# DearCaat/MHIM-MIL

Measured on AMD Instinct MI355X. Metric: patch-instances/sec through MHIM fwd+bwd, N=10k D=1024, higher is better.
Workload: dtype f32; 1 GPU; c2: MHIM(ABMIL) train step, one bag N=10000 D=1024 per GPU per step (teacher fwd + select + student fwd + bwd + Adam + EMA); rotating_bags_per_gpu=8, matrix_core_form=bf16x3, parallelism=dp1, launch=hipGraph replay, one graph per resident bag

## Files before the change

### mhim_mil_amd/csrc/select.hip

```cpp
#include "select_dev.hpp"

namespace mhimx {

#ifdef MHIMX_SEL_PROF
__device__ unsigned long long sel_prof[32];
#define SEL_STAMP(i) do { __syncthreads(); if (threadIdx.x == 0) sel_prof[i] = wall_clock64(); } while (0)
#else
#define SEL_STAMP(i)
#endif


template <bool VOTE>
__global__ __launch_bounds__(SEL_THREADS) void select_kernel(
    const float* __restrict__ score_all, int64_t N, int k, int n_sel, int largest, const int64_t* __restrict__ perm,
    const int64_t* __restrict__ other, int64_t n_other, int64_t* __restrict__ mask_ids,
    int64_t* __restrict__ len_keep_dev, int64_t* __restrict__ topk_out, uint8_t* __restrict__ flags,
    float* __restrict__ vote, int P ) {
  extern __shared__ __attribute__((aligned(16))) char smem_raw[];
  uint64_t* keys = reinterpret_cast<uint64_t*>(smem_raw);
  uint32_t* hist = reinterpret_cast<uint32_t*>(keys + P);
  uint32_t* wave_tot = hist + SEL_WAVES * 256;
  uint32_t* misc = wave_tot + SEL_WAVES;
  const int tid = threadIdx.x, lane = tid & 63, wave = tid >> 6;
  const float* score = score_all + (VOTE ? (int64_t)blockIdx.x * N : 0);
// ... 22 lines not shown
  uint32_t prefix = mx, remaining = (uint32_t)k;
  if (mn != mx) {
    const int hb = 31 - __clz(mn ^ mx);
    uint32_t fixed_mask = hb >= 31 ? 0u : ~((2u << hb) - 1u);
    prefix = mx & fixed_mask;
    int shift = hb - 7 < 0 ? 0 : hb - 7;
    while (true) {
      for (int i = tid; i < SEL_WAVES * 256; i += SEL_THREADS) hist[i] = 0;
      __syncthreads();
      for (int64_t i = tid; i < N; i += SEL_THREADS) {
        const uint32_t key = mono32(score[i], lg);
        if ((key & fixed_mask) == prefix) atomicAdd(&hist[wave * 256 + ((key >> shift) & 255u)], 1u);
      }
      __syncthreads();
      if (tid < 256) {
        uint32_t c = 0;
#pragma unroll
        for (int w = 0; w < SEL_WAVES; ++w) c += hist[w * 256 + tid];
        hist[tid] = c;
      }
      __syncthreads();
      if (tid == 0) {
        uint32_t above = 0;
        int d = 255;
        for (; d > 0; --d) {
          if (above + hist[d] >= remaining) break;
          above += hist[d];
        }
        misc[0] = (uint32_t)d;
        misc[1] = remaining - above;
      }
      __syncthreads();
      prefix |= misc[0] << shift;
      remaining = misc[1];
      fixed_mask |= 0xFFu << shift;
      __syncthreads();
      if (shift == 0) break;
      shift = shift - 8 < 0 ? 0 : shift - 8;
    }
  }
  const uint32_t T = prefix;

  if (tid == 0) misc[2] = 0;
  __syncthreads();
  uint32_t eq_base = 0;
  for (int64_t c0 = 0; c0 < N; c0 += SEL_THREADS) {
    const int64_t i = c0 + tid;
    uint32_t key = 0;
    bool gt = false, eq = false;
    if (i < N) {
      key = mono32(score[i], lg);
      gt = key > T;
      eq = key == T;
    }
    uint32_t tot;
    const uint32_t rank = block_prefix(eq, wave_tot, &tot);
    const bool take = gt || (eq && (eq_base + rank) < remaining);
    if (take) {
      const uint32_t pos = atomicAdd(&misc[2], 1u);
      keys[pos] = ((uint64_t)key << 32) | (uint64_t)(0xFFFFFFFFu - (uint32_t)i);
    }
    eq_base += tot;
  }
  __syncthreads();

  if (VOTE) {
    for (int j = tid; j < k; j += SEL_THREADS) {
      const uint32_t idx = 0xFFFFFFFFu - (uint32_t)(keys[j] & 0xFFFFFFFFull);
      atomicAdd(&vote[idx], 1.0f);
    }
    return;
  }

  for (int j = k + tid; j < P; j += SEL_THREADS) keys[j] = 0ull;
  __syncthreads();
  for (int size = 2; size <= P; size <<= 1) {
    for (int stride = size >> 1; stride > 0; stride >>= 1) {
      for (int t = tid; t < (P >> 1); t += SEL_THREADS) {
        const int lo = 2 * t - (t & (stride - 1));
        const int hi = lo + stride;
        const bool desc = ((lo & size) == 0);
        const uint64_t a = keys[lo], b = keys[hi];
        if ((a < b) == desc) { keys[lo] = b; keys[hi] = a; }
      }
      __syncthreads();
    }
  }
  if (topk_out)
    for (int j = tid; j < k; j += SEL_THREADS) topk_out[j] = (int64_t)(0xFFFFFFFFu - (uint32_t)(keys[j] & 0xFFFFFFFFull));

  for (int64_t i = tid; i < N; i += SEL_THREADS) flags[i] = 0;
  __syncthreads();
  const bool has_other = other != nullptr && n_other > 0;
  const int64_t len_keep_simple = N - n_sel;
  for (int j = tid; j < n_sel; j += SEL_THREADS) {
    const int64_t src = perm ? perm[j] : (int64_t)j;
    const int64_t idx = (int64_t)(0xFFFFFFFFu - (uint32_t)(keys[src] & 0xFFFFFFFFull));
    flags[idx] = 1;
    if (!has_other) mask_ids[len_keep_simple + j] = idx;
  }
  if (has_other)
    for (int64_t j = tid; j < n_other; j += SEL_THREADS) flags[other[j]] = 1;
  __threadfence_block();
  __syncthreads();

  uint32_t kept_base = 0;
  for (int64_t c0 = 0; c0 < N; c0 += SEL_THREADS) {
    const int64_t i = c0 + tid;
    const bool keep = (i < N) && flags[i] == 0;
    uint32_t tot;
    const uint32_t rank = block_prefix(keep, wave_tot, &tot);
    if (keep) mask_ids[kept_base + rank] = i;
    kept_base += tot;
  }
  if (has_other) {
    uint32_t m_base = 0;
    for (int64_t c0 = 0; c0 < N; c0 += SEL_THREADS) {
      const int64_t i = c0 + tid;
      const bool msk = (i < N) && flags[i] != 0;
      uint32_t tot;
      const uint32_t rank = block_prefix(msk, wave_tot, &tot);
      if (msk) mask_ids[kept_base + m_base + rank] = i;
      m_base += tot;
    }
  }
  if (tid == 0 && len_keep_dev) *len_keep_dev = (int64_t)kept_base;
}



template <int KPT, bool LEAN = false>
__global__ __launch_bounds__(SEL_THREADS) void select_small_kernel(
    const float* __restrict__ score, int N, int k, int n_sel, int largest, const int64_t* __restrict__ perm,
    const int64_t* __restrict__ other, int64_t n_other, int64_t* __restrict__ mask_ids, int64_t* __restrict__ len_keep_dev,
    int64_t* __restrict__ topk_out, int P, int use_rand, uint64_t rand_seed0, const uint64_t* __restrict__ tick, int merge_R,
    int64_t* __restrict__ rows_out,
    int64_t* __restrict__ rows_img ,
    int img_off, BagBatch bb ) {
  extern __shared__ __attribute__((aligned(16))) char smem_raw[];
  if (blockIdx.z) {
    MHIMX_BAG(score); MHIMX_BAG(perm); MHIMX_BAG(other); MHIMX_BAG(mask_ids); MHIMX_BAG(len_keep_dev); MHIMX_BAG(topk_out); MHIMX_BAG(rows_out);
    MHIMX_BAG(rows_img);
    rand_seed0 = bag_sel_seed(rand_seed0, bb);
  }
  const uint64_t rand_seed = eff_seed(rand_seed0, tick);
  uint64_t* keys = reinterpret_cast<uint64_t*>(smem_raw);
  uint64_t* sorted = keys + P;
  uint32_t* hist = reinterpret_cast<uint32_t*>(sorted + P);
  uint32_t* wave_tot = hist + SEL_COPIES * SEL_BINS;
  uint32_t* misc = wave_tot + SEL_WAVES;
  uint32_t* bitmap = misc + 8;
  uint32_t* rank = bitmap + 512;
  uint16_t* klist = reinterpret_cast<uint16_t*>(rank + P);
  uint16_t* stage = reinterpret_cast<uint16_t*>(smem_raw);
  const int tid = threadIdx.x;
  const bool lg = largest != 0;
  const int i0 = tid * KPT;

  SEL_STAMP(8);
  uint32_t key[KPT];
  bool valid[KPT];
#pragma unroll
  for (int j = 0; j < KPT; ++j) {
    valid[j] = (i0 + j) < N;
    key[j] = valid[j] ? mono32(score[i0 + j], lg) : 0u;
  }
  SEL_STAMP(0);
  for (int i = tid; i < 512; i += SEL_THREADS) bitmap[i] = 0;
  if (tid == 0) misc[2] = 0;

  uint32_t remaining, n_eq;
  const uint32_t T = radix_select_regs<KPT, false>(key, valid, (uint32_t)k, hist, wave_tot, misc, &remaining, &n_eq);

  SEL_STAMP(1);
  uint32_t eq_rank = 0;
  if (remaining != n_eq) {
    uint32_t neq = 0;
#pragma unroll
    for (int j = 0; j < KPT; ++j) neq += (valid[j] && key[j] == T) ? 1u : 0u;
    uint32_t tot;
    eq_rank = block_scan_excl(neq, wave_tot, &tot);
  }
  bool take[KPT];
  uint32_t ntake = 0;
#pragma unroll
  for (int j = 0; j < KPT; ++j) {
    bool t = valid[j] && key[j] > T;
    if (valid[j] && key[j] == T) { t = remaining == n_eq || eq_rank < remaining; ++eq_rank; }
    take[j] = t;
    ntake += t ? 1u : 0u;
  }
  {
    uint32_t tot;
    uint32_t pos = block_scan_excl(ntake, wave_tot, &tot);
#pragma unroll
    for (int j = 0; j < KPT; ++j)
      if (take[j]) keys[pos++] = ((uint64_t)key[j] << 32) | (uint64_t)(0xFFFFFFFFu - (uint32_t)(i0 + j));
  }
  __syncthreads();

  SEL_STAMP(2);
  const bool dev_rand = LEAN || (use_rand && !perm && n_sel < k);
  const uint64_t* cand = keys;
  if (LEAN || (dev_rand && !topk_out)) {
  } else if (k <= 2048) {
    for (int j = tid; j < k; j += SEL_THREADS) {
      const uint64_t mine = keys[j];
      int r = 0;
      for (int q = 0; q < k; ++q) r += keys[q] > mine ? 1 : 0;
      sorted[r] = mine;
    }
    __syncthreads();
  } else {
    for (int j = tid; j < P; j += SEL_THREADS) sorted[j] = j < k ? keys[j] : 0ull;
    __syncthreads();
    for (int size = 2; size <= P; size <<= 1)
      for (int stride = size >> 1; stride > 0; stride >>= 1) {
        for (int t = tid; t < (P >> 1); t += SEL_THREADS) {
          const int lo = 2 * t - (t & (stride - 1)), hi = lo + stride;
          const bool desc = ((lo & size) == 0);
          const uint64_t a = sorted[lo], b = sorted[hi];
          if ((a < b) == desc) { sorted[lo] = b; sorted[hi] = a; }
        }
        __syncthreads();
      }
  }
  if (!LEAN && topk_out)
    for (int j = tid; j < k; j += SEL_THREADS) topk_out[j] = (int64_t)(0xFFFFFFFFu - (uint32_t)(sorted[j] & 0xFFFFFFFFull));

  SEL_STAMP(3);
  const bool has_other = !LEAN && other != nullptr && n_other > 0;
  const int len_keep_simple = N - n_sel;
  if (dev_rand) {
    const uint32_t k0 = mix32((uint32_t)rand_seed ^ 0x9E3779B9u), k1 = mix32((uint32_t)(rand_seed >> 32) + 0x85EBCA6Bu + k0 * 0x632BE5ABu);
    const int bits = small_perm_bits((uint32_t)k);
    for (int i = tid; i < n_sel; i += SEL_THREADS) {
      const uint32_t j = feistel_small((uint32_t)i, (uint32_t)k, bits, k0, k1);
      const uint32_t idx = 0xFFFFFFFFu - (uint32_t)(cand[j] & 0xFFFFFFFFull);
      atomicOr(&bitmap[idx >> 5], 1u << (idx & 31));
      if (!LEAN && !has_other && mask_ids) mask_ids[len_keep_simple + i] = (int64_t)idx;
    }
  } else if (!LEAN) {
    for (int j = tid; j < n_sel; j += SEL_THREADS) {
      const int64_t src = perm ? perm[j] : (int64_t)j;
      const uint32_t idx = 0xFFFFFFFFu - (uint32_t)(sorted[src] & 0xFFFFFFFFull);
      atomicOr(&bitmap[idx >> 5], 1u << (idx & 31));
      if (!has_other && mask_ids) mask_ids[len_keep_simple + j] = (int64_t)idx;
    }
  }
  if (has_other)
    for (int64_t j = tid; j < n_other; j += SEL_THREADS) {
      const uint32_t idx = (uint32_t)other[j];
      atomicOr(&bitmap[idx >> 5], 1u << (idx & 31));
    }
  __syncthreads();

  SEL_STAMP(4);
  bool kv[KPT];
  uint32_t nkeep = 0;
#pragma unroll
  for (int j = 0; j < KPT; ++j) {
    const int i = i0 + j;
    kv[j] = valid[j] && !((bitmap[i >> 5] >> (i & 31)) & 1u);
    nkeep += kv[j] ? 1u : 0u;
  }
  uint32_t kept_total;
  uint32_t kpos = block_scan_excl(nkeep, wave_tot, &kept_total);
  const uint32_t kpos0 = kpos;
  if (!LEAN && mask_ids) {
#pragma unroll
    for (int j = 0; j < KPT; ++j)
      if (kv[j]) mask_ids[kpos++] = i0 + j;
    if (has_other) {
      uint32_t nm = 0;
#pragma unroll
      for (int j = 0; j < KPT; ++j) nm += (valid[j] && !kv[j]) ? 1u : 0u;
      uint32_t mt;
      uint32_t mpos = kept_total + block_scan_excl(nm, wave_tot, &mt);
#pragma unroll
      for (int j = 0; j < KPT; ++j)
        if (valid[j] && !kv[j]) mask_ids[mpos++] = i0 + j;
    }
  }
  if (!LEAN && tid == 0 && len_keep_dev) *len_keep_dev = (int64_t)kept_total;
  SEL_STAMP(5);
  if (!LEAN && !rows_out) return;

  const int Lrows = (int)kept_total;
  const int Lk = Lrows - merge_R;
  const bool partial = merge_R > 0 && merge_R < Lrows;
  if (partial) {
    uint32_t kp = kpos0;
#pragma unroll
    for (int j = 0; j < KPT; ++j)
      if (kv[j]) klist[kp++] = (uint16_t)(i0 + j);
    for (int i = tid; i < 512; i += SEL_THREADS) bitmap[i] = 0;
    __syncthreads();
    const uint32_t q1 = mix32((uint32_t)rand_seed * 0x9E3779B1u + 0xC2B2AE35u), q0 = mix32(((uint32_t)(rand_seed >> 17) ^ 0x85EBCA6Bu) + q1 * 0x632BE5ABu);
    const int bits2 = small_perm_bits((uint32_t)Lrows);
    for (int i = tid; i < merge_R; i += SEL_THREADS) {
      const uint32_t row = klist[feistel_small((uint32_t)i, (uint32_t)Lrows, bits2, q0, q1)];
      atomicOr(&bitmap[row >> 5], 1u << (row & 31));
    }
    __syncthreads();
  }
  SEL_STAMP(6);
  bool mrg[KPT];
  uint32_t nstay = 0, nmrg = 0;
#pragma unroll
  for (int j = 0; j < KPT; ++j) {
    const int i = i0 + j;
    const bool m = kv[j] && (merge_R >= Lrows || (partial && ((bitmap[i >> 5] >> (i & 31)) & 1u)));
    mrg[j] = m;
    nmrg += m ? 1u : 0u;
    nstay += (kv[j] && !m) ? 1u : 0u;
  }
  uint32_t t2;
  const uint32_t packed = block_scan_excl(nstay | (nmrg << 16), wave_tot, &t2);
  uint32_t spos = (use_rand == 2 ? (uint32_t)(Lrows - Lk) : 0u) + (packed & 0xFFFFu);
  uint32_t mpos2 = (use_rand == 2 ? 0u : (uint32_t)Lk) + (packed >> 16);
  SEL_STAMP(10);
#pragma unroll
  for (int j = 0; j < KPT; ++j) {
    if (!kv[j]) continue;
    if (mrg[j]) stage[mpos2++] = (uint16_t)(i0 + j);
    else stage[spos++] = (uint16_t)(i0 + j);
  }
  __syncthreads();
  for (int i = tid; i < Lrows; i += SEL_THREADS) rows_out[i] = (int64_t)stage[i];
  if (rows_img) {
    const int mrg_n = Lrows - Lk, stay0 = use_rand == 2 ? mrg_n : 0, mrg0 = use_rand == 2 ? 0 : Lk;
    const int end = (img_off + mrg_n + 31) / 32 * 32;
    for (int p = tid; p < end; p += SEL_THREADS)
      rows_img[p] = p < Lk ? (int64_t)stage[stay0 + p] : ((p >= img_off && p - img_off < mrg_n) ? (int64_t)stage[mrg0 + p - img_off] : (int64_t)0);
  }
  SEL_STAMP(7);
}


constexpr int SELM_MAXG = 256;
__global__ void sel_zero_kernel(uint4* __restrict__ p, int64_t n16) {
  for (int64_t i = (int64_t)blockIdx.x * blockDim.x + threadIdx.x; i < n16; i += (int64_t)gridDim.x * blockDim.x) p[i] = make_uint4(0u, 0u, 0u, 0u);
}
static int sel_zero(hipStream_t st, void* p, int64_t bytes) {
  const int64_t n16 = bytes / 16;
  int64_t blocks = cdiv(n16, 256);
  if (blocks > 1024) blocks = 1024;
  hipLaunchKernelGGL(sel_zero_kernel, dim3((unsigned)blocks), dim3(256), 0, st, (uint4*)p, n16);
  return 0;
}
struct SelMultiWs {
  uint32_t* hist;
  uint32_t* rank;
  uint32_t* selpos;
  uint32_t* blk_gt;
  uint32_t* blk_eq;
  uint32_t* blk_keep;
  uint32_t* blk_mask;
  uint32_t* state;
  uint64_t* cand;
  uint8_t* flags;
};


template <int PASS>
__global__ __launch_bounds__(SEL_THREADS) void selm_hist_kernel(const float* __restrict__ score, int64_t N, int largest, int k, SelMultiWs w) {
  __shared__ uint32_t lh[SELM_BINS];
  __shared__ __attribute__((aligned(16))) uint32_t wave_tot[SEL_WAVES];
  __shared__ uint32_t misc[8];
  const int tid = threadIdx.x;
  const bool lg = largest != 0;
  uint32_t prefix = 0, rem = 0;
  selm_prefix(w.hist, PASS, (uint32_t)k, wave_tot, misc, &prefix, &rem);
  const uint32_t fixed_mask = PASS == 0 ? 0u : (PASS == 1 ? 0xFFE00000u : 0xFFFFFC00u);
  const int shift = PASS == 0 ? 21 : (PASS == 1 ? 10 : 0);
  const uint32_t dmask = PASS == 2 ? 1023u : 2047u;
  for (int i = tid; i < SELM_BINS; i += SEL_THREADS) lh[i] = 0;
  __syncthreads();
  for (int64_t i = (int64_t)blockIdx.x * SEL_THREADS + tid; i < N; i += (int64_t)gridDim.x * SEL_THREADS) {
    const uint32_t key = mono32(score[i], lg);
    if ((key & fixed_mask) == prefix) atomicAdd(&lh[(key >> shift) & dmask], 1u);
  }
  __syncthreads();
  uint32_t* gh = w.hist + PASS * SELM_BINS;
  for (int i = tid; i < SELM_BINS; i += SEL_THREADS)
    if (lh[i]) atomicAdd(&gh[i], lh[i]);
}

__global__ __launch_bounds__(SEL_THREADS) void selm_count_kernel(const float* __restrict__ score, int64_t N, int largest, int k, int64_t chunk,
                                                                SelMultiWs w) {
  __shared__ __attribute__((aligned(16))) uint32_t wave_tot[SEL_WAVES];
  __shared__ uint32_t misc[8];
  const int tid = threadIdx.x;
  const bool lg = largest != 0;
  uint32_t T, remaining;
  selm_prefix(w.hist, 3, (uint32_t)k, wave_tot, misc, &T, &remaining);
  if (blockIdx.x == 0 && tid == 0) { w.state[0] = T; w.state[1] = remaining; }
  const int64_t b0 = (int64_t)blockIdx.x * chunk, b1 = b0 + chunk < N ? b0 + chunk : N;
  uint32_t gt = 0, eq = 0;
  for (int64_t i = b0 + tid; i < b1; i += SEL_THREADS) {
    const uint32_t key = mono32(score[i], lg);
    gt += key > T ? 1u : 0u;
    eq += key == T ? 1u : 0u;
  }
  uint32_t tg, te;
  block_scan_excl(gt, wave_tot, &tg);
  block_scan_excl(eq, wave_tot, &te);
  if (tid == 0) { w.blk_gt[blockIdx.x] = tg; w.blk_eq[blockIdx.x] = te; }
}

__global__ __launch_bounds__(SEL_THREADS) void selm_gather_kernel(const float* __restrict__ score, int64_t N, int largest, int64_t chunk,
                                                                 SelMultiWs w) {
  __shared__ __attribute__((aligned(16))) uint32_t wave_tot[SEL_WAVES];
  __shared__ uint32_t misc[8];
  const int tid = threadIdx.x, b = blockIdx.x;
  const bool lg = largest != 0;
  const uint32_t T = w.state[0], remaining = w.state[1];
  if (tid == 0) {
    uint32_t eqb = 0, pos = 0;
    for (int q = 0; q < b; ++q) {
      const uint32_t e = w.blk_eq[q];
      const uint32_t room = remaining > eqb ? remaining - eqb : 0u;
      pos += w.blk_gt[q] + (e < room ? e : room);
      eqb += e;
    }
    misc[0] = eqb;
    misc[1] = pos;
  }
  __syncthreads();
  uint32_t eq_base = misc[0], pos_base = misc[1];
  __syncthreads();
  const int64_t b0 = (int64_t)b * chunk, b1 = b0 + chunk < N ? b0 + chunk : N;
  for (int64_t c0 = b0; c0 < b1; c0 += SEL_THREADS) {
    const int64_t i = c0 + tid;
    uint32_t key = 0;
    bool gt = false, eq = false;
    if (i < b1) {
      key = mono32(score[i], lg);
      gt = key > T;
      eq = key == T;
    }
    uint32_t tot_eq, tot_take;
    const uint32_t erank = block_prefix(eq, wave_tot, &tot_eq);
    const bool take = gt || (eq && (eq_base + erank) < remaining);
    const uint32_t trank = block_prefix(take, wave_tot, &tot_take);
    if (take) w.cand[pos_base + trank] = ((uint64_t)key << 32) | (uint64_t)(0xFFFFFFFFu - (uint32_t)i);
    eq_base += tot_eq;
    pos_base += tot_take;
  }
}

constexpr int SELM_SEG = 256;
__global__ __launch_bounds__(SEL_THREADS) void selm_rank_kernel(int k, int n_sel, const int64_t* __restrict__ perm, SelMultiWs w) {
  __shared__ uint64_t seg[SELM_SEG];
  const int tid = threadIdx.x;
  const int s0 = blockIdx.y * SELM_SEG;
  for (int i = tid; i < SELM_SEG; i += SEL_THREADS) seg[i] = (s0 + i) < k ? w.cand[s0 + i] : 0ull;
  if (blockIdx.y == 0) {
    for (int j = blockIdx.x * SEL_THREADS + tid; j < n_sel; j += gridDim.x * SEL_THREADS) w.selpos[perm ? perm[j] : (int64_t)j] = (uint32_t)j + 1u;
  }
  __syncthreads();
  const int j = blockIdx.x * SEL_THREADS + tid;
  if (j >= k) return;
  const uint64_t mine = w.cand[j];
  uint32_t r = 0;
#pragma unroll 8
  for (int q = 0; q < SELM_SEG; ++q) r += seg[q] > mine ? 1u : 0u;
  if (r) atomicAdd(&w.rank[j], r);
// ... 233 lines not shown
```

### mhim_mil_amd/csrc/select_dev.hpp

```cpp
#pragma once
#include "common.hpp"

namespace mhimx {

constexpr int SEL_THREADS = 1024;
constexpr int SEL_WAVES = SEL_THREADS / 64;

MHIMX_DEV uint32_t mono32(float f, bool largest) {
  uint32_t b = __float_as_uint(f);
  b = (b & 0x80000000u) ? ~b : (b | 0x80000000u);
  return largest ? b : ~b;
}

MHIMX_DEV uint32_t block_prefix(bool pred, uint32_t* wave_tot , uint32_t* total) {
  const int lane = threadIdx.x & 63, wave = threadIdx.x >> 6;
  const unsigned long long bal = __ballot(pred);
  const uint32_t in_wave = __popcll(bal & ((1ull << lane) - 1ull));
  if (lane == 0) wave_tot[wave] = __popcll(bal);
  __syncthreads();
  uint32_t base = 0, tot = 0;
#pragma unroll
  for (int w = 0; w < SEL_WAVES; ++w) {
    const uint32_t c = wave_tot[w];
    if (w < wave) base += c;
// ... 12 lines not shown
  v += dpp_u32<0x111, 0xf>(0u, v);
  v += dpp_u32<0x112, 0xf>(0u, v);
  v += dpp_u32<0x114, 0xf>(0u, v);
  v += dpp_u32<0x118, 0xf>(0u, v);
  v += dpp_u32<0x142, 0xa>(0u, v);
  v += dpp_u32<0x143, 0xc>(0u, v);
  return v;
}
MHIMX_DEV uint32_t wave_min_u32(uint32_t v) {
  uint32_t t;
  t = dpp_u32<0xB1, 0xf>(v, v); v = t < v ? t : v;
  t = dpp_u32<0x4E, 0xf>(v, v); v = t < v ? t : v;
  t = dpp_u32<0x141, 0xf>(v, v); v = t < v ? t : v;
  t = dpp_u32<0x140, 0xf>(v, v); v = t < v ? t : v;
  t = dpp_u32<0x142, 0xa>(v, v); v = t < v ? t : v;
  t = dpp_u32<0x143, 0xc>(v, v); v = t < v ? t : v;
  return (uint32_t)__builtin_amdgcn_readlane((int)v, 63);
}
MHIMX_DEV uint32_t wave_max_u32(uint32_t v) { return ~wave_min_u32(~v); }

MHIMX_DEV void wave_tot_combine(const uint32_t* wave_tot, int wave, uint32_t* below, uint32_t* total) {
  uint32_t w[SEL_WAVES];
#pragma unroll
  for (int q = 0; q < SEL_WAVES / 4; ++q) {
    const uint4 v = reinterpret_cast<const uint4*>(wave_tot)[q];
    w[4 * q] = v.x; w[4 * q + 1] = v.y; w[4 * q + 2] = v.z; w[4 * q + 3] = v.w;
  }
  uint32_t b = 0, t = 0;
#pragma unroll
  for (int q = 0; q < SEL_WAVES; ++q) {
    b += q < wave ? w[q] : 0u;
    t += w[q];
  }
  *below = b;
  *total = t;
}

MHIMX_DEV uint32_t block_scan_excl(uint32_t v, uint32_t* wave_tot , uint32_t* total) {
  const int lane = threadIdx.x & 63, wave = threadIdx.x >> 6;
  const uint32_t inc = wave_scan_incl(v);
  if (lane == 63) wave_tot[wave] = inc;
  __syncthreads();
  uint32_t base;
  wave_tot_combine(wave_tot, wave, &base, total);
  __syncthreads();
  return base + inc - v;
}

constexpr int SEL_DIGIT = 11, SEL_BINS = 1 << SEL_DIGIT, SEL_COPIES = 4, SEL_LIST = 1024;

template <int KPT, bool FULL32>
MHIMX_DEV uint32_t radix_select_regs(const uint32_t (&key)[KPT], const bool (&valid)[KPT], uint32_t k, uint32_t* hist,
                                     uint32_t* wave_tot, uint32_t* misc, uint32_t* remaining_out, uint32_t* n_eq_out) {
  const int tid = threadIdx.x, wave = tid >> 6, lane = tid & 63;
  uint32_t prefix = 0u, fixed_mask = 0u;
  int hb = 31;
  if (!FULL32) {
    uint32_t mn = 0xFFFFFFFFu, mx = 0u;
#pragma unroll
    for (int j = 0; j < KPT; ++j)
      if (valid[j]) { mn = key[j] < mn ? key[j] : mn; mx = key[j] > mx ? key[j] : mx; }
    mn = wave_min_u32(mn);
    mx = wave_max_u32(mx);
    if (lane == 0) { hist[wave] = mn; hist[SEL_WAVES + wave] = mx; }
    __syncthreads();
#pragma unroll
    for (int q = 0; q < SEL_WAVES / 4; ++q) {
      const uint4 a = reinterpret_cast<const uint4*>(hist)[q], c = reinterpret_cast<const uint4*>(hist + SEL_WAVES)[q];
      mn = min(min(mn, min(a.x, a.y)), min(a.z, a.w));
      mx = max(max(mx, max(c.x, c.y)), max(c.z, c.w));
    }
    __syncthreads();
    const uint32_t diff = mn ^ mx;
    if (diff == 0u) {
      uint32_t nv = 0;
#pragma unroll
      for (int j = 0; j < KPT; ++j) nv += valid[j] ? 1u : 0u;
      uint32_t tot;
      block_scan_excl(nv, wave_tot, &tot);
      *remaining_out = k;
      *n_eq_out = tot;
      return mx;
    }
    hb = 31 - __clz(diff);
    fixed_mask = hb >= 31 ? 0u : ~((2u << hb) - 1u);
    prefix = mx & fixed_mask;
  }
  uint32_t remaining = k, n_eq = 0;
  int shift = hb - (SEL_DIGIT - 1) < 0 ? 0 : hb - (SEL_DIGIT - 1);
  uint32_t* copy = hist + (wave & (SEL_COPIES - 1)) * SEL_BINS;
  while (true) {
    {
      uint4* h4 = reinterpret_cast<uint4*>(hist);
      for (int i = tid; i < SEL_COPIES * SEL_BINS / 4; i += SEL_THREADS) h4[i] = make_uint4(0u, 0u, 0u, 0u);
    }
    __syncthreads();
#pragma unroll
    for (int j = 0; j < KPT; ++j)
      if (valid[j] && (key[j] & fixed_mask) == prefix) atomicAdd(&copy[(key[j] >> shift) & (SEL_BINS - 1)], 1u);
    __syncthreads();
    uint32_t c0 = 0, c1 = 0;
#pragma unroll
    for (int c = 0; c < SEL_COPIES; ++c) {
      const uint2 v = reinterpret_cast<const uint2*>(hist + c * SEL_BINS)[tid];
      c0 += v.x;
      c1 += v.y;
    }
    const uint32_t pre = wave_scan_incl(c0 + c1);
    if (lane == 63) wave_tot[wave] = pre;
    __syncthreads();
    uint32_t below, total;
    wave_tot_combine(wave_tot, wave, &below, &total);
    const uint32_t above = total - (below + pre);
    if (above < remaining && remaining <= above + c1) { misc[0] = 2u * tid + 1u; misc[1] = remaining - above; misc[3] = c1; }
    else if (above + c1 < remaining && remaining <= above + c1 + c0) { misc[0] = 2u * tid; misc[1] = remaining - above - c1; misc[3] = c0; }
    __syncthreads();
    prefix |= misc[0] << shift;
    remaining = misc[1];
    n_eq = misc[3];
    fixed_mask |= (uint32_t)(SEL_BINS - 1) << shift;
    if (shift == 0) break;
    if (n_eq <= (uint32_t)SEL_LIST) {
      if (tid == 0) misc[4] = 0;
      __syncthreads();
#pragma unroll
      for (int j = 0; j < KPT; ++j)
        if (valid[j] && (key[j] & fixed_mask) == prefix) hist[atomicAdd(&misc[4], 1u)] = key[j];
      __syncthreads();
      for (uint32_t j = tid; j < n_eq; j += SEL_THREADS) {
        const uint32_t mine = hist[j];
        uint32_t g = 0, e = 0;
        for (uint32_t q = 0; q < n_eq; ++q) {
          const uint32_t o = hist[q];
          g += o > mine ? 1u : 0u;
          e += o == mine ? 1u : 0u;
        }
        if (g < remaining && remaining <= g + e) { misc[5] = mine; misc[6] = remaining - g; misc[7] = e; }
      }
      __syncthreads();
      prefix = misc[5];
      remaining = misc[6];
      n_eq = misc[7];
      break;
    }
    __syncthreads();
    shift = shift - SEL_DIGIT < 0 ? 0 : shift - SEL_DIGIT;
  }
  __syncthreads();
  *remaining_out = remaining;
  *n_eq_out = n_eq;
  return prefix;
}

constexpr int SELM_BINS = 2048;
MHIMX_DEV void selm_find_bin(const uint32_t* __restrict__ h, uint32_t remaining, uint32_t* wave_tot, uint32_t* misc, uint32_t* bin_out,
                             uint32_t* rem_out) {
  const int tid = threadIdx.x;
  const uint2 v = reinterpret_cast<const uint2*>(h)[tid];
  uint32_t total;
  const uint32_t below = block_scan_excl(v.x + v.y, wave_tot, &total);
  const uint32_t above = total - (below + v.x + v.y);
  if (above < remaining && remaining <= above + v.y) { misc[0] = 2u * tid + 1u; misc[1] = remaining - above; }
  else if (above + v.y < remaining && remaining <= above + v.y + v.x) { misc[0] = 2u * tid; misc[1] = remaining - above - v.y; }
  __syncthreads();
  *bin_out = misc[0];
  *rem_out = misc[1];
  __syncthreads();
}

MHIMX_DEV void selm_prefix(const uint32_t* __restrict__ hist, int passes, uint32_t k, uint32_t* wave_tot, uint32_t* misc, uint32_t* prefix_out,
                           uint32_t* rem_out) {
  uint32_t prefix = 0, remaining = k, bin;
  if (passes >= 1) { selm_find_bin(hist, remaining, wave_tot, misc, &bin, &remaining); prefix = bin << 21; }
  if (passes >= 2) { selm_find_bin(hist + SELM_BINS, remaining, wave_tot, misc, &bin, &remaining); prefix |= bin << 10; }
  if (passes >= 3) { selm_find_bin(hist + 2 * SELM_BINS, remaining, wave_tot, misc, &bin, &remaining); prefix |= bin; }
  *prefix_out = prefix;
  *rem_out = remaining;
}

}
```

### mhim_mil_amd/csrc/select_many.hip

```cpp
#include "infer_tab.hpp"
#include "select_dev.hpp"

namespace mhimx {

constexpr int SM_SMALL_N = 16384, SM_SMALL_K = 4096, SM_LARGE_K = 16384;

struct SelManyTab {
  int64_t row0[MHIMX_INFER_MAX], out0[MHIMX_INFER_MAX];
  uint64_t seed[MHIMX_INFER_MAX];
  int32_t N[MHIMX_INFER_MAX], k[MHIMX_INFER_MAX], n_sel[MHIMX_INFER_MAX], merge_R[MHIMX_INFER_MAX];
};

static size_t select_many_smem(int P) { return (size_t)P * 8 + (size_t)(SEL_COPIES * SEL_BINS + SEL_WAVES + 8 + 512) * 4 + 16384 * 2; }

static int sm_pow2(int v) {
  int p = 2;
  while (p < v) p <<= 1;
  return p;
}

template <int KPT>
__global__ __launch_bounds__(SEL_THREADS) void select_many_kernel(const float* __restrict__ score_all, SelManyTab tab,
                                                                 const uint64_t* __restrict__ tick, int64_t* __restrict__ rows_all, int P,
                                                                 int merge_first) {
  extern __shared__ __attribute__((aligned(16))) char smem_raw[];
  const int bag = blockIdx.x;
  int64_t row0 = tab.row0[0], out0 = tab.out0[0];
  uint64_t seed0 = tab.seed[0];
  int N = tab.N[0], k = tab.k[0], n_sel = tab.n_sel[0], merge_R = tab.merge_R[0];
  RG_PICK(row0, tab.row0, bag) RG_PICK(out0, tab.out0, bag) RG_PICK(seed0, tab.seed, bag)
  RG_PICK(N, tab.N, bag) RG_PICK(k, tab.k, bag) RG_PICK(n_sel, tab.n_sel, bag) RG_PICK(merge_R, tab.merge_R, bag)
  const float* __restrict__ score = score_all + row0;
  int64_t* __restrict__ rows_out = rows_all + out0;
  const uint64_t rand_seed = eff_seed(seed0, tick);
  uint64_t* keys = reinterpret_cast<uint64_t*>(smem_raw);
  uint32_t* hist = reinterpret_cast<uint32_t*>(keys + P);
  uint32_t* wave_tot = hist + SEL_COPIES * SEL_BINS;
  uint32_t* misc = wave_tot + SEL_WAVES;
  uint32_t* bitmap = misc + 8;
  uint16_t* klist = reinterpret_cast<uint16_t*>(bitmap + 512);
  uint16_t* stage = reinterpret_cast<uint16_t*>(smem_raw);
  const int tid = threadIdx.x;
  const int i0 = tid * KPT;

  uint32_t key[KPT];
  bool valid[KPT];
#pragma unroll
  for (int j = 0; j < KPT; ++j) {
    valid[j] = (i0 + j) < N;
    key[j] = valid[j] ? mono32(score[i0 + j], true) : 0u;
  }
  for (int i = tid; i < 512; i += SEL_THREADS) bitmap[i] = 0;

  uint32_t remaining, n_eq;
  const uint32_t T = radix_select_regs<KPT, false>(key, valid, (uint32_t)k, hist, wave_tot, misc, &remaining, &n_eq);

  uint32_t eq_rank = 0;
  if (remaining != n_eq) {
    uint32_t neq = 0;
#pragma unroll
    for (int j = 0; j < KPT; ++j) neq += (valid[j] && key[j] == T) ? 1u : 0u;
    uint32_t tot;
    eq_rank = block_scan_excl(neq, wave_tot, &tot);
  }
  bool take[KPT];
  uint32_t ntake = 0;
#pragma unroll
  for (int j = 0; j < KPT; ++j) {
    bool t = valid[j] && key[j] > T;
    if (valid[j] && key[j] == T) { t = remaining == n_eq || eq_rank < remaining; ++eq_rank; }
    take[j] = t;
    ntake += t ? 1u : 0u;
  }
  {
    uint32_t tot;
    uint32_t pos = block_scan_excl(ntake, wave_tot, &tot);
#pragma unroll
    for (int j = 0; j < KPT; ++j)
      if (take[j]) keys[pos++] = ((uint64_t)key[j] << 32) | (uint64_t)(0xFFFFFFFFu - (uint32_t)(i0 + j));
  }
  __syncthreads();

  {
    const uint32_t k0 = mix32((uint32_t)rand_seed ^ 0x9E3779B9u), k1 = mix32((uint32_t)(rand_seed >> 32) + 0x85EBCA6Bu + k0 * 0x632BE5ABu);
    const int bits = small_perm_bits((uint32_t)k);
    for (int i = tid; i < n_sel; i += SEL_THREADS) {
      const uint32_t j = feistel_small((uint32_t)i, (uint32_t)k, bits, k0, k1);
      const uint32_t idx = 0xFFFFFFFFu - (uint32_t)(keys[j] & 0xFFFFFFFFull);
      atomicOr(&bitmap[idx >> 5], 1u << (idx & 31));
    }
  }
  __syncthreads();

  bool kv[KPT];
  uint32_t nkeep = 0;
#pragma unroll
  for (int j = 0; j < KPT; ++j) {
    const int i = i0 + j;
    kv[j] = valid[j] && !((bitmap[i >> 5] >> (i & 31)) & 1u);
    nkeep += kv[j] ? 1u : 0u;
  }
  uint32_t kept_total;
  const uint32_t kpos0 = block_scan_excl(nkeep, wave_tot, &kept_total);

  const int Lrows = (int)kept_total;
  const int Lk = Lrows - merge_R;
  const bool partial = merge_R > 0 && merge_R < Lrows;
  if (partial) {
    uint32_t kp = kpos0;
#pragma unroll
    for (int j = 0; j < KPT; ++j)
      if (kv[j]) klist[kp++] = (uint16_t)(i0 + j);
    for (int i = tid; i < 512; i += SEL_THREADS) bitmap[i] = 0;
    __syncthreads();
    const uint32_t q1 = mix32((uint32_t)rand_seed * 0x9E3779B1u + 0xC2B2AE35u), q0 = mix32(((uint32_t)(rand_seed >> 17) ^ 0x85EBCA6Bu) + q1 * 0x632BE5ABu);
    const int bits2 = small_perm_bits((uint32_t)Lrows);
    for (int i = tid; i < merge_R; i += SEL_THREADS) {
      const uint32_t row = klist[feistel_small((uint32_t)i, (uint32_t)Lrows, bits2, q0, q1)];
      atomicOr(&bitmap[row >> 5], 1u << (row & 31));
    }
    __syncthreads();
  }
  bool mrg[KPT];
  uint32_t nstay = 0, nmrg = 0;
#pragma unroll
  for (int j = 0; j < KPT; ++j) {
    const int i = i0 + j;
    const bool m = kv[j] && (merge_R >= Lrows || (partial && ((bitmap[i >> 5] >> (i & 31)) & 1u)));
    mrg[j] = m;
    nmrg += m ? 1u : 0u;
    nstay += (kv[j] && !m) ? 1u : 0u;
  }
  uint32_t t2;
  const uint32_t packed = block_scan_excl(nstay | (nmrg << 16), wave_tot, &t2);
  uint32_t spos = (merge_first ? (uint32_t)(Lrows - Lk) : 0u) + (packed & 0xFFFFu);
  uint32_t mpos2 = (merge_first ? 0u : (uint32_t)Lk) + (packed >> 16);
#pragma unroll
  for (int j = 0; j < KPT; ++j) {
    if (!kv[j]) continue;
    if (mrg[j]) stage[mpos2++] = (uint16_t)(i0 + j);
    else stage[spos++] = (uint16_t)(i0 + j);
  }
  __syncthreads();
  for (int i = tid; i < Lrows; i += SEL_THREADS) rows_out[i] = (int64_t)stage[i];
}

int select_large_rows(hipStream_t st, const float* score, int64_t N, int64_t k, int64_t n_sel, uint64_t seed, const uint64_t* tick, int64_t merge_R,
                      int64_t* rows_out, int merge_first, const SelLargeWs& w) {
  const int64_t len_keep = N - n_sel, Lk = len_keep - merge_R;
  if (int r = mhimx_random_perm(st, k, seed + 0x51ED270Bull, tick, nullptr, w.perm)) return r;
  if (int r = mhimx_select_mask(st, score, N, k, n_sel, 1, n_sel < k ? w.perm : nullptr, nullptr, 0, w.ids, w.lk, nullptr, w.sel_ws, w.sel_ws_bytes))
    return r;
  if (!merge_first) return mhimx_random_perm(st, len_keep, seed ^ 0x3C6EF372FE94F82Bull, tick, w.ids, rows_out);
  if (int r = mhimx_random_perm(st, len_keep, seed ^ 0x3C6EF372FE94F82Bull, tick, w.ids, w.rows)) return r;
  if (merge_R) MHIMX_HIP(hipMemcpyAsync(rows_out, w.rows + Lk, (size_t)merge_R * 8, hipMemcpyDeviceToDevice, st));
  if (Lk) MHIMX_HIP(hipMemcpyAsync(rows_out + merge_R, w.rows, (size_t)Lk * 8, hipMemcpyDeviceToDevice, st));
  return 0;
}

int select_bags_check(const char* who, int32_t n_bags, const mhimx_select_bag* bags) {
  MHIMX_CHECK_ARG(n_bags >= 1 && n_bags <= MHIMX_INFER_MAX, "%s: n_bags=%d must be in 1..%d", who, n_bags, MHIMX_INFER_MAX);
  MHIMX_CHECK_ARG(bags, "%s: null bag table", who);
  for (int b = 0; b < n_bags; ++b) {
    const mhimx_select_bag& q = bags[b];
    MHIMX_CHECK_ARG(q.N >= 1 && q.N <= MHIMX_STEP_MAX_ROWS, "%s: bag %d: N=%lld must be in 1..%d", who, b, (long long)q.N, MHIMX_STEP_MAX_ROWS);
    const int64_t kcap = q.N <= SM_SMALL_N ? SM_SMALL_K : SM_LARGE_K, kmax = q.N < kcap ? q.N : kcap;
    MHIMX_CHECK_ARG(q.k >= 1 && q.k <= kmax, "%s: bag %d: k=%lld must be in 1..%lld (min(N, %lld) for a bag %s 16384 rows)", who, b, (long long)q.k,
                    (long long)kmax, (long long)kcap, q.N <= SM_SMALL_N ? "of up to" : "above");
    MHIMX_CHECK_ARG(q.n_sel >= 0 && q.n_sel <= q.k, "%s: bag %d: n_sel=%lld must be in 0..k", who, b, (long long)q.n_sel);
    MHIMX_CHECK_ARG(q.merge_R >= 0 && q.merge_R <= q.N - q.n_sel, "%s: bag %d: merge_R=%lld must be in 0..N - n_sel", who, b, (long long)q.merge_R);
    MHIMX_CHECK_ARG(q.row0 >= 0 && q.out0 >= 0, "%s: bag %d: row0 / out0 must be >= 0", who, b);
  }
  for (int b = 1; b < n_bags; ++b)
    for (int a = 0; a < b; ++a) {
      const int64_t a0 = bags[a].out0, a1 = a0 + bags[a].N - bags[a].n_sel, b0 = bags[b].out0, b1 = b0 + bags[b].N - bags[b].n_sel;
      MHIMX_CHECK_ARG(!(a0 < a1 && b0 < b1 && a0 < b1 && b0 < a1), "%s: bag %d: its output rows [%lld, %lld) overlap those of bag %d", who, b, (long long)b0, (long long)b1, a);
    }
  return 0;
}

struct SmLay { int64_t perm, ids, rows, sel_ws, sel_ws_bytes, total; };
static SmLay sm_layout(int32_t n_bags, const mhimx_select_bag* bags) {
  int64_t perm_n = 0, ids_n = 0, rows_n = 0, sel_b = 0;
  for (int b = 0; b < n_bags; ++b) {
    const mhimx_select_bag& q = bags[b];
    if (q.N <= SM_SMALL_N) continue;
    auto up = [](int64_t& a, int64_t v) { if (v > a) a = v; };
    up(perm_n, q.k); up(ids_n, q.N); up(rows_n, q.N - q.n_sel); up(sel_b, mhimx_select_ws_bytes(q.N));
  }
  SmLay l;
  Arena ar(nullptr, 0);
  ar.take<char>(256);
  l.perm = ar.off; ar.take<int64_t>(perm_n);
  l.ids = ar.off; ar.take<int64_t>(ids_n);
  l.rows = ar.off; ar.take<int64_t>(rows_n);
  l.sel_ws_bytes = sel_b; l.sel_ws = ar.off; ar.take<char>(sel_b);
  l.total = ar.off;
  return l;
}

int select_rows_many_launch(hipStream_t st, const float* score, int32_t n_bags, const mhimx_select_bag* bags, const uint64_t* tick,
                            int64_t* rows_out, const SelLargeWs& w, int merge_first) {
  SelManyTab tab = {};
  int n_small = 0, kmax = 1;
  int64_t nmax = 0;
  for (int b = 0; b < n_bags; ++b) {
    const mhimx_select_bag& q = bags[b];
    if (q.N > SM_SMALL_N) continue;
    tab.row0[n_small] = q.row0; tab.out0[n_small] = q.out0; tab.seed[n_small] = q.seed;
    tab.N[n_small] = (int32_t)q.N; tab.k[n_small] = (int32_t)q.k; tab.n_sel[n_small] = (int32_t)q.n_sel; tab.merge_R[n_small] = (int32_t)q.merge_R;
    ++n_small;
    if (q.N > nmax) nmax = q.N;
    if (q.k > kmax) kmax = (int)q.k;
  }
  if (n_small) {
    const int P = sm_pow2(kmax);
    const size_t sm = select_many_smem(P);
    MHIMX_ONCE_PER_DEVICE(
        MHIMX_HIP(hipFuncSetAttribute((const void*)select_many_kernel<16>, hipFuncAttributeMaxDynamicSharedMemorySize, (int)select_many_smem(SM_SMALL_K)));
        MHIMX_HIP(hipFuncSetAttribute((const void*)select_many_kernel<10>, hipFuncAttributeMaxDynamicSharedMemorySize, (int)select_many_smem(SM_SMALL_K)));
        MHIMX_HIP(hipFuncSetAttribute((const void*)select_many_kernel<4>, hipFuncAttributeMaxDynamicSharedMemorySize, (int)select_many_smem(SM_SMALL_K))));
#define MHIMX_SEL_MANY(KPT) \
    hipLaunchKernelGGL(select_many_kernel<KPT>, dim3((unsigned)n_small), dim3(SEL_THREADS), sm, st, score, tab, tick, rows_out, P, merge_first ? 1 : 0)
    if (nmax <= 4096) MHIMX_SEL_MANY(4);
    else if (nmax <= 10240) MHIMX_SEL_MANY(10);
    else MHIMX_SEL_MANY(16);
#undef MHIMX_SEL_MANY
    MHIMX_LAUNCH_CHECK();
  }
  for (int b = 0; b < n_bags; ++b) {
    const mhimx_select_bag& q = bags[b];
    if (q.N <= SM_SMALL_N) continue;
    if (int r = select_large_rows(st, score + q.row0, q.N, q.k, q.n_sel, q.seed, tick, q.merge_R, rows_out + q.out0, merge_first, w)) return r;
  }
  return 0;
}

}

using namespace mhimx;

extern "C" int64_t mhimx_select_rows_many_ws_bytes(int32_t n_bags, const mhimx_select_bag* bags) {
  if (select_bags_check("mhimx_select_rows_many_ws_bytes", n_bags, bags)) return -1;
  return sm_layout(n_bags, bags).total;
}

extern "C" int mhimx_select_rows_many(void* stream, const float* score, int32_t n_bags, const mhimx_select_bag* bags, const uint64_t* tick,
                                      int64_t* rows_out, void* ws, int64_t ws_bytes, int32_t merge_first) {
  const char* who = "mhimx_select_rows_many";
  if (select_bags_check(who, n_bags, bags)) return -1;
  MHIMX_CHECK_ARG(score && rows_out, "%s: null score / rows_out", who);
  const SmLay l = sm_layout(n_bags, bags);
  if (rg_check_ws(who, ws, ws_bytes, l.total)) return -1;
  char* base = static_cast<char*>(ws);
  SelLargeWs w;
  w.lk = reinterpret_cast<int64_t*>(base);
  w.perm = reinterpret_cast<int64_t*>(base + l.perm);
  w.ids = reinterpret_cast<int64_t*>(base + l.ids);
  w.rows = reinterpret_cast<int64_t*>(base + l.rows);
  w.sel_ws = base + l.sel_ws;
  w.sel_ws_bytes = l.sel_ws_bytes;
  return select_rows_many_launch((hipStream_t)stream, score, n_bags, bags, tick, rows_out, w, merge_first);
}
```

Baseline: 33.48 million patch-instances/s.

## Precompute random pick bitmaps by rank in lean select path, overlapping score loads

In the lean select kernels, the random picks are drawn before the radix select, as bitmaps indexed by candidate rank and kept-row rank. This removes the shared-memory key array write, the klist staging and several block barriers with atomic passes that came after the threshold was known. The score loads are issued first and the Feistel draws run while those loads are in flight. The result depends on the candidate order by index equalling the old keys-array order, and it adds a barrier inside draw_pick_bitmaps.

Result: no change. 33.72 million patch-instances/s, median of 2 (+0.7%).

```diff
diff --git a/mhim_mil_amd/csrc/select.hip b/mhim_mil_amd/csrc/select.hip
--- a/mhim_mil_amd/csrc/select.hip
+++ b/mhim_mil_amd/csrc/select.hip
@@ -198,6 +198,7 @@
   uint32_t* bitmap = misc + 8;
   uint32_t* rank = bitmap + 512;
   uint16_t* klist = reinterpret_cast<uint16_t*>(rank + P);
+  uint32_t* candbits = reinterpret_cast<uint32_t*>(klist);
   uint16_t* stage = reinterpret_cast<uint16_t*>(smem_raw);
   const int tid = threadIdx.x;
   const bool lg = largest != 0;
@@ -206,14 +207,28 @@
   SEL_STAMP(8);
   uint32_t key[KPT];
   bool valid[KPT];
-#pragma unroll
-  for (int j = 0; j < KPT; ++j) {
-    valid[j] = (i0 + j) < N;
-    key[j] = valid[j] ? mono32(score[i0 + j], lg) : 0u;
+  if constexpr (LEAN) {
+    float sc[KPT];
+#pragma unroll
+    for (int j = 0; j < KPT; ++j) {
+      valid[j] = (i0 + j) < N;
+      sc[j] = load_global_f32(score + (valid[j] ? i0 + j : N - 1));
+    }
+    draw_pick_bitmaps(candbits, bitmap, rand_seed, N, k, n_sel, merge_R);
+#pragma unroll
+    for (int j = 0; j < KPT; ++j) key[j] = valid[j] ? mono32(sc[j], lg) : 0u;
+  } else {
+#pragma unroll
+    for (int j = 0; j < KPT; ++j) {
+      valid[j] = (i0 + j) < N;
+      key[j] = valid[j] ? mono32(score[i0 + j], lg) : 0u;
+    }
   }
   SEL_STAMP(0);
-  for (int i = tid; i < 512; i += SEL_THREADS) bitmap[i] = 0;
-  if (tid == 0) misc[2] = 0;
+  if constexpr (!LEAN) {
+    for (int i = tid; i < 512; i += SEL_THREADS) bitmap[i] = 0;
+    if (tid == 0) misc[2] = 0;
+  }
 
   uint32_t remaining, n_eq;
   const uint32_t T = radix_select_regs<KPT, false>(key, valid, (uint32_t)k, hist, wave_tot, misc, &remaining, &n_eq);
@@ -236,79 +251,94 @@
     take[j] = t;
     ntake += t ? 1u : 0u;
   }
+  bool kv[KPT];
+  uint32_t nkeep = 0;
   {
     uint32_t tot;
     uint32_t pos = block_scan_excl(ntake, wave_tot, &tot);
-#pragma unroll
-    for (int j = 0; j < KPT; ++j)
-      if (take[j]) keys[pos++] = ((uint64_t)key[j] << 32) | (uint64_t)(0xFFFFFFFFu - (uint32_t)(i0 + j));
-  }
-  __syncthreads();
+    if constexpr (LEAN) {
+#pragma unroll
+      for (int j = 0; j < KPT; ++j) {
+        const bool masked = take[j] && pick_bit(candbits, pos);
+        pos += take[j] ? 1u : 0u;
+        kv[j] = valid[j] && !masked;
+        nkeep += kv[j] ? 1u : 0u;
+      }
+    } else {
+#pragma unroll
+      for (int j = 0; j < KPT; ++j)
+        if (take[j]) keys[pos++] = ((uint64_t)key[j] << 32) | (uint64_t)(0xFFFFFFFFu - (uint32_t)(i0 + j));
+    }
+  }
+  if constexpr (!LEAN) __syncthreads();
 
   SEL_STAMP(2);
-  const bool dev_rand = LEAN || (use_rand && !perm && n_sel < k);
-  const uint64_t* cand = keys;
-  if (LEAN || (dev_rand && !topk_out)) {
-  } else if (k <= 2048) {
-    for (int j = tid; j < k; j += SEL_THREADS) {
-      const uint64_t mine = keys[j];
-      int r = 0;
-      for (int q = 0; q < k; ++q) r += keys[q] > mine ? 1 : 0;
-      sorted[r] = mine;
-    }
+  const bool has_other = !LEAN && other != nullptr && n_other > 0;
+  if constexpr (!LEAN) {
+    const bool dev_rand = use_rand && !perm && n_sel < k;
+    const uint64_t* cand = keys;
+    if (dev_rand && !topk_out) {
+    } else if (k <= 2048) {
+      for (int j = tid; j < k; j += SEL_THREADS) {
+        const uint64_t mine = keys[j];
+        int r = 0;
+        for (int q = 0; q < k; ++q) r += keys[q] > mine ? 1 : 0;
+        sorted[r] = mine;
+      }
+      __syncthreads();
+    } else {
+      for (int j = tid; j < P; j += SEL_THREADS) sorted[j] = j < k ? keys[j] : 0ull;
+      __syncthreads();
+      for (int size = 2; size <= P; size <<= 1)
+        for (int stride = size >> 1; stride > 0; stride >>= 1) {
+          for (int t = tid; t < (P >> 1); t += SEL_THREADS) {
+            const int lo = 2 * t - (t & (stride - 1)), hi = lo + stride;
+            const bool desc = ((lo & size) == 0);
+            const uint64_t a = sorted[lo], b = sorted[hi];
+            if ((a < b) == desc) { sorted[lo] = b; sorted[hi] = a; }
+          }
+          __syncthreads();
+        }
+    }
+    if (topk_out)
+      for (int j = tid; j < k; j += SEL_THREADS) topk_out[j] = (int64_t)(0xFFFFFFFFu - (uint32_t)(sorted[j] & 0xFFFFFFFFull));
+
+    SEL_STAMP(3);
+    const int len_keep_simple = N - n_sel;
+    if (dev_rand) {
+      const uint32_t k0 = mix32((uint32_t)rand_seed ^ 0x9E3779B9u), k1 = mix32((uint32_t)(rand_seed >> 32) + 0x85EBCA6Bu + k0 * 0x632BE5ABu);
+      const int bits = small_perm_bits((uint32_t)k);
+      for (int i = tid; i < n_sel; i += SEL_THREADS) {
+        const uint32_t j = feistel_small((uint32_t)i, (uint32_t)k, bits, k0, k1);
+        const uint32_t idx = 0xFFFFFFFFu - (uint32_t)(cand[j] & 0xFFFFFFFFull);
+        atomicOr(&bitmap[idx >> 5], 1u << (idx & 31));
+        if (!has_other && mask_ids) mask_ids[len_keep_simple + i] = (int64_t)idx;
+      }
+    } else {
+      for (int j = tid; j < n_sel; j += SEL_THREADS) {
+        const int64_t src = perm ? perm[j] : (int64_t)j;
+        const uint32_t idx = 0xFFFFFFFFu - (uint32_t)(sorted[src] & 0xFFFFFFFFull);
+        atomicOr(&bitmap[idx >> 5], 1u << (idx & 31));
+        if (!has_other && mask_ids) mask_ids[len_keep_simple + j] = (int64_t)idx;
+      }
+    }
+    if (has_other)
+      for (int64_t j = tid; j < n_other; j += SEL_THREADS) {
+        const uint32_t idx = (uint32_t)other[j];
+        atomicOr(&bitmap[idx >> 5], 1u << (idx & 31));
+      }
     __syncthreads();
+
+    SEL_STAMP(4);
+#pragma unroll
+    for (int j = 0; j < KPT; ++j) {
+      const int i = i0 + j;
+      kv[j] = valid[j] && !((bitmap[i >> 5] >> (i & 31)) & 1u);
+      nkeep += kv[j] ? 1u : 0u;
+    }
   } else {
-    for (int j = tid; j < P; j += SEL_THREADS) sorted[j] = j < k ? keys[j] : 0ull;
-    __syncthreads();
-    for (int size = 2; size <= P; size <<= 1)
-      for (int stride = size >> 1; stride > 0; stride >>= 1) {
-        for (int t = tid; t < (P >> 1); t += SEL_THREADS) {
-          const int lo = 2 * t - (t & (stride - 1)), hi = lo + stride;
-          const bool desc = ((lo & size) == 0);
-          const uint64_t a = sorted[lo], b = sorted[hi];
-          if ((a < b) == desc) { sorted[lo] = b; sorted[hi] = a; }
-        }
-        __syncthreads();
-      }
-  }
-  if (!LEAN && topk_out)
-    for (int j = tid; j < k; j += SEL_THREADS) topk_out[j] = (int64_t)(0xFFFFFFFFu - (uint32_t)(sorted[j] & 0xFFFFFFFFull));
-
-  SEL_STAMP(3);
-  const bool has_other = !LEAN && other != nullptr && n_other > 0;
-  const int len_keep_simple = N - n_sel;
-  if (dev_rand) {
-    const uint32_t k0 = mix32((uint32_t)rand_seed ^ 0x9E3779B9u), k1 = mix32((uint32_t)(rand_seed >> 32) + 0x85EBCA6Bu + k0 * 0x632BE5ABu);
-    const int bits = small_perm_bits((uint32_t)k);
-    for (int i = tid; i < n_sel; i += SEL_THREADS) {
-      const uint32_t j = feistel_small((uint32_t)i, (uint32_t)k, bits, k0, k1);
-      const uint32_t idx = 0xFFFFFFFFu - (uint32_t)(cand[j] & 0xFFFFFFFFull);
-      atomicOr(&bitmap[idx >> 5], 1u << (idx & 31));
-      if (!LEAN && !has_other && mask_ids) mask_ids[len_keep_simple + i] = (int64_t)idx;
-    }
-  } else if (!LEAN) {
-    for (int j = tid; j < n_sel; j += SEL_THREADS) {
-      const int64_t src = perm ? perm[j] : (int64_t)j;
-      const uint32_t idx = 0xFFFFFFFFu - (uint32_t)(sorted[src] & 0xFFFFFFFFull);
-      atomicOr(&bitmap[idx >> 5], 1u << (idx & 31));
-      if (!has_other && mask_ids) mask_ids[len_keep_simple + j] = (int64_t)idx;
-    }
-  }
-  if (has_other)
-    for (int64_t j = tid; j < n_other; j += SEL_THREADS) {
-      const uint32_t idx = (uint32_t)other[j];
-      atomicOr(&bitmap[idx >> 5], 1u << (idx & 31));
-    }
-  __syncthreads();
-
-  SEL_STAMP(4);
-  bool kv[KPT];
-  uint32_t nkeep = 0;
-#pragma unroll
-  for (int j = 0; j < KPT; ++j) {
-    const int i = i0 + j;
-    kv[j] = valid[j] && !((bitmap[i >> 5] >> (i & 31)) & 1u);
-    nkeep += kv[j] ? 1u : 0u;
+    SEL_STAMP(3);
+    SEL_STAMP(4);
   }
   uint32_t kept_total;
   uint32_t kpos = block_scan_excl(nkeep, wave_tot, &kept_total);
@@ -335,31 +365,44 @@
   const int Lrows = (int)kept_total;
   const int Lk = Lrows - merge_R;
   const bool partial = merge_R > 0 && merge_R < Lrows;
-  if (partial) {
-    uint32_t kp = kpos0;
-#pragma unroll
-    for (int j = 0; j < KPT; ++j)
-      if (kv[j]) klist[kp++] = (uint16_t)(i0 + j);
-    for (int i = tid; i < 512; i += SEL_THREADS) bitmap[i] = 0;
-    __syncthreads();
-    const uint32_t q1 = mix32((uint32_t)rand_seed * 0x9E3779B1u + 0xC2B2AE35u), q0 = mix32(((uint32_t)(rand_seed >> 17) ^ 0x85EBCA6Bu) + q1 * 0x632BE5ABu);
-    const int bits2 = small_perm_bits((uint32_t)Lrows);
-    for (int i = tid; i < merge_R; i += SEL_THREADS) {
-      const uint32_t row = klist[feistel_small((uint32_t)i, (uint32_t)Lrows, bits2, q0, q1)];
-      atomicOr(&bitmap[row >> 5], 1u << (row & 31));
-    }
-    __syncthreads();
-  }
-  SEL_STAMP(6);
   bool mrg[KPT];
   uint32_t nstay = 0, nmrg = 0;
-#pragma unroll
-  for (int j = 0; j < KPT; ++j) {
-    const int i = i0 + j;
-    const bool m = kv[j] && (merge_R >= Lrows || (partial && ((bitmap[i >> 5] >> (i & 31)) & 1u)));
-    mrg[j] = m;
-    nmrg += m ? 1u : 0u;
-    nstay += (kv[j] && !m) ? 1u : 0u;
+  if constexpr (LEAN) {
+    SEL_STAMP(6);
+    uint32_t q = kpos0;
+#pragma unroll
+    for (int j = 0; j < KPT; ++j) {
+      const bool m = kv[j] && (merge_R >= Lrows || (partial && pick_bit(bitmap, q)));
+      q += kv[j] ? 1u : 0u;
+      mrg[j] = m;
+      nmrg += m ? 1u : 0u;
+      nstay += (kv[j] && !m) ? 1u : 0u;
+    }
+  } else {
+    if (partial) {
+      uint32_t kp = kpos0;
+#pragma unroll
+      for (int j = 0; j < KPT; ++j)
+        if (kv[j]) klist[kp++] = (uint16_t)(i0 + j);
+      for (int i = tid; i < 512; i += SEL_THREADS) bitmap[i] = 0;
+      __syncthreads();
+      const uint32_t q1 = mix32((uint32_t)rand_seed * 0x9E3779B1u + 0xC2B2AE35u), q0 = mix32(((uint32_t)(rand_seed >> 17) ^ 0x85EBCA6Bu) + q1 * 0x632BE5ABu);
+      const int bits2 = small_perm_bits((uint32_t)Lrows);
+      for (int i = tid; i < merge_R; i += SEL_THREADS) {
+        const uint32_t row = klist[feistel_small((uint32_t)i, (uint32_t)Lrows, bits2, q0, q1)];
+        atomicOr(&bitmap[row >> 5], 1u << (row & 31));
+      }
+      __syncthreads();
+    }
+    SEL_STAMP(6);
+#pragma unroll
+    for (int j = 0; j < KPT; ++j) {
+      const int i = i0 + j;
+      const bool m = kv[j] && (merge_R >= Lrows || (partial && ((bitmap[i >> 5] >> (i & 31)) & 1u)));
+      mrg[j] = m;
+      nmrg += m ? 1u : 0u;
+      nstay += (kv[j] && !m) ? 1u : 0u;
+    }
   }
   uint32_t t2;
   const uint32_t packed = block_scan_excl(nstay | (nmrg << 16), wave_tot, &t2);
diff --git a/mhim_mil_amd/csrc/select_dev.hpp b/mhim_mil_amd/csrc/select_dev.hpp
--- a/mhim_mil_amd/csrc/select_dev.hpp
+++ b/mhim_mil_amd/csrc/select_dev.hpp
@@ -188,6 +188,27 @@
   return prefix;
 }
 
+constexpr int SEL_CANDBITS = 128, SEL_POSBITS = 512;
+MHIMX_DEV void draw_pick_bitmaps(uint32_t* candbits, uint32_t* posbits, uint64_t rand_seed, int N, int k, int n_sel, int merge_R) {
+  const int tid = threadIdx.x;
+  if (tid < SEL_POSBITS) posbits[tid] = 0;
+  else if (tid < SEL_POSBITS + SEL_CANDBITS) candbits[tid - SEL_POSBITS] = 0;
+  __syncthreads();
+  const int Lrows = N - n_sel;
+  const int n2 = (merge_R > 0 && merge_R < Lrows) ? merge_R : 0;
+  const uint32_t k0 = mix32((uint32_t)rand_seed ^ 0x9E3779B9u), k1 = mix32((uint32_t)(rand_seed >> 32) + 0x85EBCA6Bu + k0 * 0x632BE5ABu);
+  const uint32_t q1 = mix32((uint32_t)rand_seed * 0x9E3779B1u + 0xC2B2AE35u), q0 = mix32(((uint32_t)(rand_seed >> 17) ^ 0x85EBCA6Bu) + q1 * 0x632BE5ABu);
+  const int bits = small_perm_bits((uint32_t)k), bits2 = small_perm_bits((uint32_t)Lrows);
+  for (int i = tid; i < n_sel + n2; i += SEL_THREADS) {
+    const bool second = i >= n_sel;
+    const uint32_t p = feistel_small((uint32_t)(second ? i - n_sel : i), (uint32_t)(second ? Lrows : k), second ? bits2 : bits, second ? q0 : k0,
+                                     second ? q1 : k1);
+    atomicOr(&(second ? posbits : candbits)[p >> 5], 1u << (p & 31));
+  }
+}
+MHIMX_DEV float load_global_f32(const float* p) { return *(const __attribute__((address_space(1))) float*)p; }
+MHIMX_DEV bool pick_bit(const uint32_t* bits, uint32_t p) { return (bits[p >> 5] >> (p & 31)) & 1u; }
+
 constexpr int SELM_BINS = 2048;
 MHIMX_DEV void selm_find_bin(const uint32_t* __restrict__ h, uint32_t remaining, uint32_t* wave_tot, uint32_t* misc, uint32_t* bin_out,
                              uint32_t* rem_out) {
diff --git a/mhim_mil_amd/csrc/select_many.hip b/mhim_mil_amd/csrc/select_many.hip
--- a/mhim_mil_amd/csrc/select_many.hip
+++ b/mhim_mil_amd/csrc/select_many.hip
@@ -33,24 +33,26 @@
   const float* __restrict__ score = score_all + row0;
   int64_t* __restrict__ rows_out = rows_all + out0;
   const uint64_t rand_seed = eff_seed(seed0, tick);
-  uint64_t* keys = reinterpret_cast<uint64_t*>(smem_raw);
-  uint32_t* hist = reinterpret_cast<uint32_t*>(keys + P);
+  uint32_t* hist = reinterpret_cast<uint32_t*>(smem_raw + (size_t)P * 8);
   uint32_t* wave_tot = hist + SEL_COPIES * SEL_BINS;
   uint32_t* misc = wave_tot + SEL_WAVES;
-  uint32_t* bitmap = misc + 8;
-  uint16_t* klist = reinterpret_cast<uint16_t*>(bitmap + 512);
+  uint32_t* posbits = misc + 8;
+  uint32_t* candbits = posbits + SEL_POSBITS;
   uint16_t* stage = reinterpret_cast<uint16_t*>(smem_raw);
   const int tid = threadIdx.x;
   const int i0 = tid * KPT;
 
+  float sc[KPT];
   uint32_t key[KPT];
   bool valid[KPT];
 #pragma unroll
   for (int j = 0; j < KPT; ++j) {
     valid[j] = (i0 + j) < N;
-    key[j] = valid[j] ? mono32(score[i0 + j], true) : 0u;
-  }
-  for (int i = tid; i < 512; i += SEL_THREADS) bitmap[i] = 0;
+    sc[j] = load_global_f32(score + (valid[j] ? i0 + j : N - 1));
+  }
+  draw_pick_bitmaps(candbits, posbits, rand_seed, N, k, n_sel, merge_R);
+#pragma unroll
+  for (int j = 0; j < KPT; ++j) key[j] = valid[j] ? mono32(sc[j], true) : 0u;
 
   uint32_t remaining, n_eq;
   const uint32_t T = radix_select_regs<KPT, false>(key, valid, (uint32_t)k, hist, wave_tot, misc, &remaining, &n_eq);
@@ -72,33 +74,19 @@
     take[j] = t;
     ntake += t ? 1u : 0u;
   }
+
+  bool kv[KPT];
+  uint32_t nkeep = 0;
   {
     uint32_t tot;
     uint32_t pos = block_scan_excl(ntake, wave_tot, &tot);
 #pragma unroll
-    for (int j = 0; j < KPT; ++j)
-      if (take[j]) keys[pos++] = ((uint64_t)key[j] << 32) | (uint64_t)(0xFFFFFFFFu - (uint32_t)(i0 + j));
-  }
-  __syncthreads();
-
-  {
-    const uint32_t k0 = mix32((uint32_t)rand_seed ^ 0x9E3779B9u), k1 = mix32((uint32_t)(rand_seed >> 32) + 0x85EBCA6Bu + k0 * 0x632BE5ABu);
-    const int bits = small_perm_bits((uint32_t)k);
-    for (int i = tid; i < n_sel; i += SEL_THREADS) {
-      const uint32_t j = feistel_small((uint32_t)i, (uint32_t)k, bits, k0, k1);
-      const uint32_t idx = 0xFFFFFFFFu - (uint32_t)(keys[j] & 0xFFFFFFFFull);
-      atomicOr(&bitmap[idx >> 5], 1u << (idx & 31));
+    for (int j = 0; j < KPT; ++j) {
+      const bool masked = take[j] && pick_bit(candbits, pos);
+      pos += take[j] ? 1u : 0u;
+      kv[j] = valid[j] && !masked;
+      nkeep += kv[j] ? 1u : 0u;
     }
-  }
-  __syncthreads();
-
-  bool kv[KPT];
-  uint32_t nkeep = 0;
-#pragma unroll
-  for (int j = 0; j < KPT; ++j) {
-    const int i = i0 + j;
-    kv[j] = valid[j] && !((bitmap[i >> 5] >> (i & 31)) & 1u);
-    nkeep += kv[j] ? 1u : 0u;
   }
   uint32_t kept_total;
   const uint32_t kpos0 = block_scan_excl(nkeep, wave_tot, &kept_total);
@@ -106,30 +94,18 @@
   const int Lrows = (int)kept_total;
   const int Lk = Lrows - merge_R;
   const bool partial = merge_R > 0 && merge_R < Lrows;
-  if (partial) {
-    uint32_t kp = kpos0;
-#pragma unroll
-    for (int j = 0; j < KPT; ++j)
-      if (kv[j]) klist[kp++] = (uint16_t)(i0 + j);
-    for (int i = tid; i < 512; i += SEL_THREADS) bitmap[i] = 0;
-    __syncthreads();
-    const uint32_t q1 = mix32((uint32_t)rand_seed * 0x9E3779B1u + 0xC2B2AE35u), q0 = mix32(((uint32_t)(rand_seed >> 17) ^ 0x85EBCA6Bu) + q1 * 0x632BE5ABu);
-    const int bits2 = small_perm_bits((uint32_t)Lrows);
-    for (int i = tid; i < merge_R; i += SEL_THREADS) {
-      const uint32_t row = klist[feistel_small((uint32_t)i, (uint32_t)Lrows, bits2, q0, q1)];
-      atomicOr(&bitmap[row >> 5], 1u << (row & 31));
-    }
-    __syncthreads();
-  }
   bool mrg[KPT];
   uint32_t nstay = 0, nmrg = 0;
-#pragma unroll
-  for (int j = 0; j < KPT; ++j) {
-    const int i = i0 + j;
-    const bool m = kv[j] && (merge_R >= Lrows || (partial && ((bitmap[i >> 5] >> (i & 31)) & 1u)));
-    mrg[j] = m;
-    nmrg += m ? 1u : 0u;
-    nstay += (kv[j] && !m) ? 1u : 0u;
+  {
+    uint32_t q = kpos0;
+#pragma unroll
+    for (int j = 0; j < KPT; ++j) {
+      const bool m = kv[j] && (merge_R >= Lrows || (partial && pick_bit(posbits, q)));
+      q += kv[j] ? 1u : 0u;
+      mrg[j] = m;
+      nmrg += m ? 1u : 0u;
+      nstay += (kv[j] && !m) ? 1u : 0u;
+    }
   }
   uint32_t t2;
   const uint32_t packed = block_scan_excl(nstay | (nmrg << 16), wave_tot, &t2);
```
